# ndlongvn/MM-DTI

Measured on AMD Instinct MI355X. Metric: molecules/sec fwd+bwd (InfoNCE fine-tune), higher is better.
Workload: dtype fp16 forward / bf16 backward GEMM operands, fp32 accumulation

## Files before the change

include/mmdti_hip.h:

```cpp
#ifndef MMDTI_HIP_H
#define MMDTI_HIP_H

#ifdef __cplusplus
extern "C" {
#endif

typedef void* mmdti_stream_t;

#define MMDTI_OK 0
#define MMDTI_ERR_INVALID 1
#define MMDTI_ERR_LAUNCH 2

#define MMDTI_ACT_NONE 0
#define MMDTI_ACT_GELU 1
#define MMDTI_ACT_GELU_BWD 2
#define MMDTI_ACT_GELU_G 4
#define MMDTI_ACT_MUL_AUX 5

#define MMDTI_DT_F32 0
#define MMDTI_DT_BF16 1
#define MMDTI_DT_F32_ATOMIC 2
#define MMDTI_DT_F16 3
#define MMDTI_DT_AB_F16 16
#define MMDTI_DT_B_F16 32
// ... 113 lines not shown
                         long long arena_bytes, long long stats_bytes, void* ws, long long ws_bytes, long long dw_slab_bytes,
                         int fwd_f16);


int mmdti_layernorm_fwd(mmdti_stream_t stream, const float* x, const float* gamma, const float* beta, float eps,
                        int rows, int D, float* y_f32, void* y_bf16, float* mean, float* rstd,
                        const unsigned char* row_zero, float drop_p, unsigned long long seed, unsigned int site,
                        int y16_f16 );
int mmdti_layernorm_bwd(mmdti_stream_t stream, const void* dy, int dy_dtype, const float* dy_add, const float* x, const float* gamma,
                        const float* mean, const float* rstd, int rows, int D, const float* dres, float* dx,
                        float* dgamma, float* dbeta, const unsigned char* row_zero, float drop_p,
                        unsigned long long seed, unsigned int site, void* dx_bf16, float drop2_p, unsigned int site2,
                        float* dx_colsum);

int mmdti_colsum_bf16(mmdti_stream_t stream, const void* x_bf16, int rows, int cols, int ld, float* out);
int mmdti_cast_f32_bf16(mmdti_stream_t stream, const float* x, void* y_bf16, long long n, float drop_p,
                        unsigned long long seed, unsigned int site);
int mmdti_cast_bf16_f32(mmdti_stream_t stream, const void* x_bf16, float* y, long long n);
int mmdti_cast_f32_f16(mmdti_stream_t stream, const float* x, void* y_f16, long long n, float drop_p, unsigned long long seed,
                       unsigned int site);
int mmdti_cast_f16_bf16(mmdti_stream_t stream, const void* x_f16, int rows, int cols, int ldx, void* y_bf16);
int mmdti_dropout_f32(mmdti_stream_t stream, const float* x, float* y, long long n, float drop_p,
                      unsigned long long seed, unsigned int site);
int mmdti_axpy_f32(mmdti_stream_t stream, const float* x, float* y, long long n, float a);

int mmdti_embedding_fwd(mmdti_stream_t stream, const long long* ids, const float* table, long long n, int D,
                        int vocab, float* out, int accumulate);
int mmdti_embedding_bwd(mmdti_stream_t stream, const long long* ids, const float* dout, long long n, int D,
                        int vocab, long long padding_idx, float* dtable);
int mmdti_embedding_fwd3(mmdti_stream_t stream, const long long* ids_a, const float* table_a, int vocab_a, const long long* ids_b,
                         const float* table_b, int vocab_b, const long long* ids_c, const float* table_c, int vocab_c, long long n, int D,
                         float* out);
int mmdti_onehot_bf16(mmdti_stream_t stream, const long long* ids, long long n, int vocab, int ld, long long padding_idx,
                      void* out_bf16);
int mmdti_roberta_position_ids(mmdti_stream_t stream, const long long* ids, int B, int L, long long pad_idx,
                               long long* out);

int mmdti_gbf_features_fwd(mmdti_stream_t stream, const float* dist, const long long* edge_type, const float* mul,
                           const float* bias, const float* means, const float* stds, long long P, int K, int E,
                           void* feat_bf16);
int mmdti_gbf_features_bwd(mmdti_stream_t stream, const float* dist, const long long* edge_type, const float* mul,
                           const float* bias, const float* means, const float* stds, long long P, int K, int E,
                           const void* dfeat_bf16, float* dmul, float* dbias, float* dmeans, float* dstds);
int mmdti_gbf_bias_fwd(mmdti_stream_t stream, const float* dist, const void* edge_type,
                       int edge_bytes , const float* mul,
                       const float* bias, const float* means, const float* stds, const void* w1_bf16, const float* b1,
// ... 129 lines not shown
```

mm-dti_amd/csrc/elementwise.hip:

```cpp
#include "common.h"
#include <stdarg.h>
#include <stdio.h>

namespace mmdti {

static thread_local char g_err[512] = "";
void set_error(const char* fmt, ...) {
  va_list ap;
  va_start(ap, fmt);
  vsnprintf(g_err, sizeof(g_err), fmt, ap);
  va_end(ap);
}

static inline int grid_for(long long n, int per_block) {
  long long b = (n + per_block - 1) / per_block;
  if (b > 256 * 16) b = 256 * 16;
  if (b < 1) b = 1;
  return (int)b;
}

__device__ __forceinline__ bf16_t f2h16(float f) { return f2h_sat(f); }

template <bool F16>
__global__ __launch_bounds__(256) void cast_f32_bf16_kernel(const float* __restrict__ x, bf16_t* __restrict__ y,
// ... 32 lines not shown
    const int c = (int)(i - row * cols8) * 8;
    const uint4 u = *reinterpret_cast<const uint4*>(x + row * ldx + c);
    const uint32_t w[4] = {u.x, u.y, u.z, u.w};
    uint32_t o[4];
#pragma unroll
    for (int e = 0; e < 4; ++e) {
      const float lo = (float)__builtin_bit_cast(_Float16, (uint16_t)(w[e] & 0xffffu)), hi = (float)__builtin_bit_cast(_Float16, (uint16_t)(w[e] >> 16));
      o[e] = (uint32_t)f2bf(lo) | ((uint32_t)f2bf(hi) << 16);
    }
    *reinterpret_cast<uint4*>(y + row * (long long)cols8 * 8 + c) = make_uint4(o[0], o[1], o[2], o[3]);
  }
}

__global__ __launch_bounds__(256) void cast_bf16_f32_kernel(const bf16_t* __restrict__ x, float* __restrict__ y, long long n) {
  for (long long i = (long long)blockIdx.x * 256 + threadIdx.x; i < n; i += (long long)gridDim.x * 256) y[i] = bf2f(x[i]);
}

__global__ __launch_bounds__(256) void dropout_f32_kernel(const float* __restrict__ x, float* __restrict__ y, long long n,
                                                          uint32_t thresh, float dscale, uint64_t seed, uint32_t site) {
  for (long long i = (long long)blockIdx.x * 256 + threadIdx.x; i < n; i += (long long)gridDim.x * 256) {
    float o = x[i];
    if (thresh) o = dropout_keep(seed, site, (uint64_t)i, thresh) ? o * dscale : 0.f;
    y[i] = o;
  }
}

__global__ __launch_bounds__(256) void axpy_kernel(const float* __restrict__ x, float* __restrict__ y, long long n, float a) {
  for (long long i = (long long)blockIdx.x * 256 + threadIdx.x; i < n; i += (long long)gridDim.x * 256) y[i] += a * x[i];
}

__global__ __launch_bounds__(256) void gelu_bf16_kernel(const bf16_t* __restrict__ u, bf16_t* __restrict__ y, long long n) {
  for (long long i = (long long)blockIdx.x * 256 + threadIdx.x; i < n; i += (long long)gridDim.x * 256)
    y[i] = f2bf(gelu_erf(bf2f(u[i])));
}

__global__ __launch_bounds__(256) void colsum_bf16_kernel(const bf16_t* __restrict__ x, int rows, int cols, int ld,
                                                          float* __restrict__ out) {
  __shared__ float red[8][256 + 8];
  const int cc = threadIdx.x & 31, rl = threadIdx.x >> 5;
  const int c0 = blockIdx.x * 256 + cc * 8;
  float acc[8] = {0, 0, 0, 0, 0, 0, 0, 0};
  if (c0 < cols) {
    const int rstep = gridDim.y * 8;
    int r = blockIdx.y * 8 + rl;
    if (c0 + 8 <= cols) {
      for (; r + 3 * rstep < rows; r += 4 * rstep) {
// ... 546 lines not shown
                     (bf16_t*)y_bf16, n8);
  MMDTI_LAUNCH_CHECK();
  return MMDTI_OK;
}

extern "C" int mmdti_cast_bf16_f32(mmdti_stream_t stream, const void* x_bf16, float* y, long long n) {
  MMDTI_REQUIRE(x_bf16 && y && n > 0, "cast_bf16_f32: bad arguments");
  hipLaunchKernelGGL(cast_bf16_f32_kernel, dim3(grid_for(n, 256)), dim3(256), 0, (hipStream_t)stream,
                     (const bf16_t*)x_bf16, y, n);
  MMDTI_LAUNCH_CHECK();
  return MMDTI_OK;
}

extern "C" int mmdti_dropout_f32(mmdti_stream_t stream, const float* x, float* y, long long n, float drop_p,
                                 unsigned long long seed, unsigned int site) {
  MMDTI_REQUIRE(x && y && n > 0, "dropout_f32: bad arguments");
  DROP_SETUP("dropout_f32");
  hipLaunchKernelGGL(dropout_f32_kernel, dim3(grid_for(n, 256)), dim3(256), 0, (hipStream_t)stream, x, y, n, th, sc,
                     (uint64_t)seed, (uint32_t)site);
  MMDTI_LAUNCH_CHECK();
  return MMDTI_OK;
}

extern "C" int mmdti_axpy_f32(mmdti_stream_t stream, const float* x, float* y, long long n, float a) {
  MMDTI_REQUIRE(x && y && n > 0, "axpy_f32: bad arguments");
  hipLaunchKernelGGL(axpy_kernel, dim3(grid_for(n, 256)), dim3(256), 0, (hipStream_t)stream, x, y, n, a);
  MMDTI_LAUNCH_CHECK();
  return MMDTI_OK;
}

extern "C" int mmdti_gelu_fwd_bf16(mmdti_stream_t stream, const void* u_bf16, void* y_bf16, long long n) {
  MMDTI_REQUIRE(u_bf16 && y_bf16 && n > 0, "gelu_fwd_bf16: bad arguments");
  hipLaunchKernelGGL(gelu_bf16_kernel, dim3(grid_for(n, 256)), dim3(256), 0, (hipStream_t)stream,
                     (const bf16_t*)u_bf16, (bf16_t*)y_bf16, n);
  MMDTI_LAUNCH_CHECK();
  return MMDTI_OK;
}

extern "C" int mmdti_colsum_bf16(mmdti_stream_t stream, const void* x_bf16, int rows, int cols, int ld, float* out) {
  MMDTI_REQUIRE(x_bf16 && out && rows > 0 && cols > 0 && ld >= cols, "colsum_bf16: bad arguments");
  MMDTI_REQUIRE(ld % 8 == 0 && aligned16(x_bf16), "colsum_bf16: ld%%8 and 16-byte alignment required");
  int gy = cdiv(rows, 8 * 8);
  if (gy > 1024) gy = 1024;
  hipLaunchKernelGGL(colsum_bf16_kernel, dim3(cdiv(cols, 256), gy), dim3(256), 0, (hipStream_t)stream,
                     (const bf16_t*)x_bf16, rows, cols, ld, out);
  MMDTI_LAUNCH_CHECK();
// ... 239 lines not shown
```

mm-dti_amd/mmdti_hip/functional.py:

```python
from __future__ import annotations

import ctypes
import os
import weakref

import math
from types import SimpleNamespace
from typing import List, Optional

import torch

from . import ops, paths
from .ops import BF16, F32
from .runtime import fused_views, wbf16, wfwd, gbuf, dropout_state, notify_grads_ready
from .freeze import layer_trainable, plan_tower, trainable_flags


def _lin_bwd_params(dy_bf16, x_bf16, weight, bias, rows=None, bias_done=False):
    gw = gbuf(weight)
    gb = gbuf(bias) if (bias is not None and not bias_done) else None
    if gw is not None:
        ops.linear_bwd_weight(dy_bf16, x_bf16, gw, rows=rows, db=gb if (gb is not None and gb.numel() == gw.shape[0]) else None)
        if gb is not None and gb.numel() == gw.shape[0]:
            gb = None
# ... 1018 lines not shown
    @staticmethod
    def backward(ctx, dout):
        st, mod = ctx.st, ctx.mod
        if getattr(st, "consumed", False):
            raise ops.MMDTIError("RobertaEncoderFn: backward through the same forward twice (retain_graph) is not supported")
        st.consumed = True
        B, Lq, D = st.B, st.Lq, st.D
        dx = dout.contiguous().view(st.Mq, D)
        if st.stack is not None:
            dx = _bert_stack_bwd(st, dx)
            notify_grads_ready(st.stack.T.params)
            st.stack = None
        plan = st.plan
        for li, layer, L in zip(range(len(st.layers) - 1, -1, -1), reversed(list(mod.layers)), reversed(st.layers)):
            if li < plan.lowest:
                L.__dict__.clear()
                continue
            dx, _ = _bert_layer_bwd(st, L, dx, st.seed, (plan.needs_dx(li), False))
            L.__dict__.clear()
            notify_grads_ready(layer.parameters())
        if not plan.below:
            _join_stream_after_backward()
            return None, None, None, None, None, None
        de = ops.layernorm_bwd(dx, st.e.view(st.Mq, D), mod.emb_ln_w, st.em, st.er, gbuf(mod.emb_ln_w), gbuf(mod.emb_ln_b),
                               drop_p=st.p_hid, seed=st.seed, site=st.site_emb)
        cfg = mod.cfg
        de16 = ops.cast_bf16(de)
        for ids, w, pad in ((st.ids, mod.word, cfg.pad_idx), (st.pos, mod.position, cfg.pad_idx), (None, mod.token_type, -1)):
            g = gbuf(w)
            if g is not None:
                if ids is None:
                    ids = st.ids if w.shape[0] == 1 else torch.zeros_like(st.ids)
                ops.embedding_bwd_gemm(ids, de16, g, pad)
        notify_grads_ready(mod.embeddings.parameters())
        _join_stream_after_backward()
        return None, None, None, None, None, None


class CrossLayerFn(torch.autograd.Function):

    @staticmethod
    def forward(ctx, s1, s2, key_add, layer, cfg, training, packs=None, anchor=None):
        seed = dropout_state.next_seed()
        sites = _Sites()
        p_hid = cfg.hidden_dropout if training else 0.0
        p_att = cfg.attn_dropout if training else 0.0
        if packs is not None:
            vl = ops.AttnVarlen(packs[0], packs[1])
            D = s1.shape[-1]
            st = SimpleNamespace(B=packs[0].B, Lq=vl.Lq, Lk=vl.Lk, D=D, seed=seed, Mq=vl.q_rows, Mk=vl.k_rows, vl=vl)
        else:
            B, Lq, D = s1.shape
            Lk = s2.shape[1]
            st = SimpleNamespace(B=B, Lq=Lq, Lk=Lk, D=D, seed=seed, Mq=B * Lq, Mk=B * Lk, vl=None)
        s1c = s1.contiguous().view(st.Mq, D)
        s1_16 = ops.cast_act16(s1c)
        s2_16 = ops.cast_act16(s2.contiguous().view(st.Mk, D))
        L, out32, _ = _bert_layer_fwd(st, s1c, s1_16, s2_16, None if key_add is None else key_add.contiguous(), bert_weights(layer), cfg.heads,
                                      p_hid, p_att, cfg.ln_eps, seed, sites, False)
        if any(ctx.needs_input_grad):
            ctx.st, ctx.L, ctx.layer = st, L, layer
        ctx.shapes = (s1.shape, s2.shape)
        return out32.view(s1.shape)

    @staticmethod
    def backward(ctx, dout):
        st, L = ctx.st, ctx.L
        want = ctx.needs_input_grad[:2]
        ds1, ds2 = _bert_layer_bwd(st, L, dout.contiguous().view(st.Mq, st.D), st.seed, want)
        L.__dict__.clear()
        notify_grads_ready(ctx.layer.parameters())
        return (None if ds1 is None else ds1.view(ctx.shapes[0]), None if ds2 is None else ds2.view(ctx.shapes[1]), None, None, None, None, None,
                None)


class DropoutFn(torch.autograd.Function):

    @staticmethod
    def forward(ctx, x, p, training):
        if not training or p == 0.0:
            ctx.p = 0.0
            return x
        ctx.p, ctx.seed = p, dropout_state.next_seed()
        return ops.dropout_f32(x.contiguous(), p, ctx.seed, 1)

    @staticmethod
    def backward(ctx, d):
        if ctx.p == 0.0:
            return d, None, None
        return ops.dropout_f32(d.contiguous(), ctx.p, ctx.seed, 1), None, None


def _pad8(n):
    return (n + 7) // 8 * 8


class InfoNCEFn(torch.autograd.Function):

    @staticmethod
    def forward(ctx, query, positive, mod, training, gather, reduce_scatter, row0, packs=None, anchor=None):
        if packs is not None:
            B, D = packs[0].B, query.shape[-1]
            Nq, Np = packs[0].M, packs[1].M
            if not (POOL_THEN_PROJECT and mod.info_proj_query[0].weight.shape[0] % 8 == 0 and mod.info_proj_positive[0].weight.shape[0] % 8 == 0):
                raise ops.MMDTIError("InfoNCEFn: packed rows need the pool-then-project form (hidden width % 8 == 0)")
        else:
            B, Nq, D = query.shape
            Np = positive.shape[1]
        d = mod.d_l
        ldp = _pad8(d)
        seed = dropout_state.next_seed()
        p = mod.embed_dropout if training else 0.0
        st = SimpleNamespace(B=B, Nq=Nq, Np=Np, D=D, d=d, ldp=ldp, seed=seed, p=p)
        dev = query.device

        def proj(x, seq, n, dropout_p, site, pack=None):
            L = SimpleNamespace()
            rows = B * n if pack is None else pack.M
            L.x16 = ops.cast_act16(x.contiguous().view(rows, D), dropout_p, seed, site)
            L.u = torch.empty(rows, seq[0].weight.shape[0], device=dev, dtype=BF16)
            h = ops.linear_fwd(L.x16, wfwd(seq[0].weight), seq[0].bias, act=ops.ACT_GELU_FWD, aux_out=L.u, out_dtype=BF16)
            Hd = h.shape[1]
            if pack is not None:
                L.hbar = ops.seq_mean_packed_fwd(h, pack, Hd, Hd)
                L.mean = ops.linear_f32_fwd(L.hbar, seq[2].weight.detach(), seq[2].bias.detach())
                L.h = None
                return L
            if POOL_THEN_PROJECT and Hd % 8 == 0:
                L.hbar = ops.seq_mean_fwd(h, B, n, Hd, Hd)
                L.mean = ops.linear_f32_fwd(L.hbar, seq[2].weight.detach(), seq[2].bias.detach())
                L.h = None
                return L
            L.h = h
            pr = torch.zeros(B * n, ldp, device=dev, dtype=BF16)
# ... 22 lines not shown
    @staticmethod
    def backward(ctx, dloss):
        st, mod = ctx.st, ctx.mod
        B, d, ldp = st.B, st.d, st.ldp
        dq = ops.l2norm_bwd(st.dqh, st.qh, st.qinv)
        dk = ops.l2norm_bwd(st.dkh, st.kh, st.kinv)
        dboth = torch.cat((dq, dk), dim=1)
        if ctx.rs is not None:
            dboth = ctx.rs(dboth)
        dboth = (dboth * dloss).contiguous()

        def proj_bwd(L, dmean, seq, n, dropout_p, site, want_dx, pack=None):
            if L.h is None:
                gw, gb = gbuf(seq[2].weight), gbuf(seq[2].bias)
                dhbar = ops.linear_f32_bwd(L.hbar, seq[2].weight.detach(), None, dmean.contiguous(), gw, gb)
                Hd = L.hbar.shape[1]
                if pack is not None:
                    du = ops.seq_mean_packed_bwd(dhbar, pack, Hd, Hd, aux=L.u, aux_mode=1 if ops.GELU_SAVE_GRAD else 2)
                else:
                    du = ops.seq_mean_bwd(dhbar, B, n, Hd, Hd, aux=L.u, aux_mode=1 if ops.GELU_SAVE_GRAD else 2)
                _lin_bwd_params(du, L.x16, seq[0].weight, seq[0].bias)
                if not want_dx:
                    return None
                dx = ops.linear_bwd_input(du, wbf16(seq[0].weight), out_dtype=F32)
                if dropout_p > 0:
                    dx = ops.dropout_f32(dx, dropout_p, st.seed, site)
                return dx
            dpr = ops.seq_mean_bwd(dmean.contiguous(), B, n, d, ldp)
            gw = gbuf(seq[2].weight)
            if gw is not None:
                ops.linear_bwd_weight(dpr, L.h, gw)
            gb = gbuf(seq[2].bias)
            if gb is not None:
                ops.colsum(dpr, gb, cols=d)
            du = ops.gemm(dpr, wbf16(seq[2].weight), M=B * n, N=L.h.shape[1], K=d, lda=ldp, ldb=seq[2].weight.shape[1], transB=True,
                          act=ops.ACT_GELU_DX, aux_in=L.u)
            _lin_bwd_params(du, L.x16, seq[0].weight, seq[0].bias)
            if not want_dx:
                return None
            dx = ops.linear_bwd_input(du, wbf16(seq[0].weight), out_dtype=F32)
            if dropout_p > 0:
                dx = ops.dropout_f32(dx, dropout_p, st.seed, site)
            return dx

        pk = st.packs
        dxq = proj_bwd(st.Lq, dboth[:, :d], mod.info_proj_query, st.Nq, st.p, 1, ctx.needs_input_grad[0], None if pk is None else pk[0])
        dxp = proj_bwd(st.Lp, dboth[:, d:], mod.info_proj_positive, st.Np, 0.0, 2, ctx.needs_input_grad[1], None if pk is None else pk[1])
        notify_grads_ready(mod.parameters())
        if pk is not None:
            return dxq, dxp, None, None, None, None, None, None, None
        return (None if dxq is None else dxq.view(B, st.Nq, st.D), None if dxp is None else dxp.view(B, st.Np, st.D), None, None, None, None, None, None,
                None)


class InfoNCELossFn(torch.autograd.Function):

    @staticmethod
    def forward(ctx, q, k, temperature):
        B, d = q.shape
        qh, qinv = ops.l2norm_fwd(q.contiguous())
        kh, kinv = ops.l2norm_fwd(k.contiguous())
        loss = torch.zeros(1, device=q.device, dtype=F32)
        dqh, dkh = torch.zeros_like(qh), torch.zeros_like(kh)
        ops.infonce_dir(qh, kh, 0, B, temperature, loss, dqh, dkh)
        ops.infonce_dir(kh, qh, 0, B, temperature, loss, dkh, dqh)
        ctx.sv = (qh, qinv, kh, kinv, dqh, dkh)
        return (loss / (2.0 * B)).view(())

    @staticmethod
    def backward(ctx, dl):
        qh, qinv, kh, kinv, dqh, dkh = ctx.sv
        return ops.l2norm_bwd(dqh, qh, qinv) * dl, ops.l2norm_bwd(dkh, kh, kinv) * dl, None


class CTLossFn(torch.autograd.Function):
# ... 106 lines not shown
```

mm-dti_amd/mmdti_hip/models/bert_layers.py:

```python
import json
import os
from types import SimpleNamespace

import torch
import torch.nn as nn

from ..unicore_compat import LayerNorm
from ..functional import RobertaEncoderFn, CrossLayerFn
from ..freeze import grad_anchor


class _SelfAttnParams(nn.Module):
    def __init__(self, dim):
        super().__init__()
        self.query = nn.Linear(dim, dim)
        self.key = nn.Linear(dim, dim)
        self.value = nn.Linear(dim, dim)


class _SelfOutputParams(nn.Module):
    def __init__(self, in_dim, dim, eps):
        super().__init__()
        self.dense = nn.Linear(in_dim, dim)
        self.LayerNorm = LayerNorm(dim, eps=eps)
# ... 11 lines not shown
        super().__init__()
        self.dense = nn.Linear(dim, ffn)


class BertLayerParams(nn.Module):
    def __init__(self, dim, ffn, eps):
        super().__init__()
        self.attention = _AttentionParams(dim, eps)
        self.intermediate = _IntermediateParams(dim, ffn)
        self.output = _SelfOutputParams(ffn, dim, eps)


class BertCrossEncoder(nn.Module):

    def __init__(self, config, layer_num):
        super().__init__()
        if config.hidden_act != "gelu":
            raise NotImplementedError("only hidden_act='gelu' is on the MM-DTI path")
        self.cfg = SimpleNamespace(heads=config.num_attention_heads, ln_eps=config.layer_norm_eps,
                                   hidden_dropout=config.hidden_dropout_prob, attn_dropout=config.attention_probs_dropout_prob)
        self.layer = nn.ModuleList([BertLayerParams(config.hidden_size, config.intermediate_size, config.layer_norm_eps)
                                    for _ in range(layer_num)])

    def forward(self, s1_hidden_states, s2_hidden_states, s2_attention_mask, output_all_encoded_layers=True, packs=None):
        if packs is None:
            B, Lk = s2_hidden_states.shape[0], s2_hidden_states.shape[1]
            key_add = s2_attention_mask.reshape(B, Lk).float()
        else:
            key_add = None
        outs = []
        for layer in self.layer:
            s1_hidden_states = CrossLayerFn.apply(s1_hidden_states.float(), s2_hidden_states.float(), key_add, layer, self.cfg, self.training, packs,
                                                  grad_anchor(layer.parameters()))
            if output_all_encoded_layers:
                outs.append(s1_hidden_states)
        if not output_all_encoded_layers:
            outs.append(s1_hidden_states)
        return outs


class _RobertaEmbeddings(nn.Module):
    def __init__(self, cfg):
        super().__init__()
        self.word_embeddings = nn.Embedding(cfg.vocab, cfg.dim, padding_idx=cfg.pad_idx)
        self.position_embeddings = nn.Embedding(cfg.max_pos, cfg.dim, padding_idx=cfg.pad_idx)
        self.token_type_embeddings = nn.Embedding(cfg.type_vocab, cfg.dim)
        self.LayerNorm = LayerNorm(cfg.dim, eps=cfg.ln_eps)


class _RobertaEncoder(nn.Module):
    def __init__(self, cfg):
        super().__init__()
        self.layer = nn.ModuleList([BertLayerParams(cfg.dim, cfg.ffn, cfg.ln_eps) for _ in range(cfg.layers)])


class _Pooler(nn.Module):
# ... 80 lines not shown
```

mm-dti_amd/mmdti_hip/models/infonce.py:

```python
import torch
from torch import nn

from ..functional import InfoNCEFn, InfoNCELossFn
from ..freeze import grad_anchor


class InfoNCE(nn.Module):
    def __init__(self, bert_output_size, graph_ouput_size, temperature=0.1, reduction='mean', negative_mode='unpaired'):
        super().__init__()
        self.temperature = temperature
        self.reduction = reduction
        self.negative_mode = negative_mode
        self.orig_d_l = bert_output_size
        self.orig_d_av = graph_ouput_size
        self.d_l, self.d_av = 50, 50
        self.embed_dropout = 0.1
        self.training = True
        self.info_proj_query = nn.Sequential(nn.Linear(self.orig_d_l, self.orig_d_l), nn.GELU(), nn.Linear(self.orig_d_l, self.d_l))
        self.info_proj_positive = nn.Sequential(nn.Linear(self.orig_d_av, self.orig_d_av), nn.GELU(), nn.Linear(self.orig_d_av, self.d_av))
        self._gather = None
        self._reduce_scatter = None
        self._row0 = 0

    def set_global_negatives(self, gather, reduce_scatter, row0):
        self._gather, self._reduce_scatter, self._row0 = gather, reduce_scatter, int(row0)

    def forward(self, query, positive_key, negative_keys=None, packs=None):
        if packs is not None:
            if negative_keys is not None or self.reduction != 'mean' or query.dim() != 2 or positive_key.dim() != 2 or packs[0].B != packs[1].B:
                raise ValueError('packed rows: <query> / <positive_key> must be [rows, dim] with one packing each, implicit negatives.')
            return InfoNCEFn.apply(query.float(), positive_key.float(), self, self.training, self._gather, self._reduce_scatter, self._row0, packs,
                                   grad_anchor(self.parameters()))
        if negative_keys is not None:
            raise ValueError("explicit negative_keys are unreachable in the reference (infonce.py:98 raises); not supported")
        if self.reduction != 'mean':
            raise ValueError("only reduction='mean' is on the MM-DTI path")
        if self.orig_d_l == self.d_l or self.orig_d_av == self.d_av:
            raise ValueError("identity projection (input width == 50) is not on the MM-DTI path")
        if query.dim() != 3 or positive_key.dim() != 3:
            raise ValueError('<query> and <positive_key> must be [batch, seq, dim] token representations.')
        if len(query) != len(positive_key):
            raise ValueError('<query> and <positive_key> must must have the same number of samples.')
        return InfoNCEFn.apply(query.float(), positive_key.float(), self, self.training, self._gather, self._reduce_scatter, self._row0, None,
                               grad_anchor(self.parameters()))


def info_nce(query, positive_key, negative_keys=None, temperature=0.1, reduction='mean', negative_mode='unpaired'):
    if query.dim() != 2:
        raise ValueError('<query> must have 2 dimensions.')
    if positive_key.dim() != 2:
        raise ValueError('<positive_key> must have 2 dimensions.')
    if negative_keys is not None:
        if negative_mode == 'unpaired' and negative_keys.dim() != 2:
            raise ValueError("<negative_keys> must have 2 dimensions if <negative_mode> == 'unpaired'.")
        if negative_mode == 'paired' and negative_keys.dim() != 3:
            raise ValueError("<negative_keys> must have 3 dimensions if <negative_mode> == 'paired'.")
    if len(query) != len(positive_key):
        raise ValueError('<query> and <positive_key> must must have the same number of samples.')
    if negative_keys is not None:
        if negative_mode == 'paired' and len(query) != len(negative_keys):
            raise ValueError("If negative_mode == 'paired', then <negative_keys> must have the same number of samples as <query>.")
    if query.shape[-1] != positive_key.shape[-1]:
        raise ValueError('Vectors of <query> and <positive_key> should have the same number of components.')
    if negative_keys is not None:
        if query.shape[-1] != negative_keys.shape[-1]:
            raise ValueError('Vectors of <query> and <negative_keys> should have the same number of components.')
        raise ValueError("explicit negative_keys: the reference's symmetric cross-entropy (infonce.py:98) raises for "
# ... 5 lines not shown
```

mm-dti_amd/mmdti_hip/models/mm_model.py:

```python
from __future__ import annotations

import argparse
import itertools
import os
from types import SimpleNamespace

import torch
import torch.nn as nn

from ..unicore_compat import Dictionary, init_bert_params, get_activation_fn
from ..functional import PairBiasFn, PairCompactFn, EmbeddingFn, DropoutFn, MaskedPoolFn, LinearF32Fn
from .. import ops
from ..freeze import grad_anchor
from ..collate import right_pad, collate_batch
from ..packing import PackedRows

PAIR_RAGGED = os.environ.get("MMDTI_PAIR_RAGGED", "1") != "0"
from .transformers import TransformerEncoderWithPair
from .bert_layers import BertCrossEncoder, RobertaTower
from .infonce import InfoNCE
from .fds import FDS

BACKBONE = {'transformer': TransformerEncoderWithPair}


def pad_1d_tokens(values, pad_idx):
    return right_pad(values, pad_idx)


def pad_2d(values, pad_idx):
    return right_pad(values, pad_idx, square=True)


def pad_coords(values, pad_idx):
    return right_pad(values, pad_idx, tail=(3,))

# ... 51 lines not shown

def fds_config():
    return SimpleNamespace(feature_dim=512, bucket_num=20, bucket_start=0, start_update=0, start_smooth=1, kernel='gaussian',
                           ks=5, sigma=1, momentum=0.9, col_data="expt", raw_data="")


def crossmodal_config():
    return SimpleNamespace(attention_probs_dropout_prob=0.2, gradient_checkpointing=False, hidden_act="gelu",
                           hidden_dropout_prob=0.3, hidden_size=512, initializer_range=0.02, intermediate_size=2048,
                           layer_norm_eps=1e-12, max_position_embeddings=512, num_attention_heads=16, num_hidden_layers=12,
                           position_embedding_type="absolute")


class CrossAttentionModel(nn.Module):

    def __init__(self, cross_cfg, num_layers=1):
        super().__init__()
        self.text_attention = BertCrossEncoder(cross_cfg, num_layers)
        self.graph_attention = BertCrossEncoder(cross_cfg, num_layers)
        self.dropout = nn.Dropout(cross_cfg.hidden_dropout_prob)
        self.two_streams = os.environ.get("MMDTI_CROSS_TWO_STREAMS", "1") != "0"
        self._stream = None

    def forward(self, text_embeddings, graph_embeddings, text_mask, graph_mask, packs=None):
        text_embeddings = DropoutFn.apply(text_embeddings, self.dropout.p, self.training)
        graph_embeddings = DropoutFn.apply(graph_embeddings, self.dropout.p, self.training)
        if packs is not None:
            rev = (packs[1], packs[0])
            if self.two_streams and text_embeddings.is_cuda:
                main = torch.cuda.current_stream()
                if self._stream is None:
                    self._stream = torch.cuda.Stream()
                st = self._stream
                st.wait_stream(main)
                with torch.cuda.stream(st):
                    text_to_graph = self.text_attention(text_embeddings, graph_embeddings, None, packs=packs)[-1]
                for t in (text_embeddings, graph_embeddings):
                    t.record_stream(st)
                graph_to_text = self.graph_attention(graph_embeddings, text_embeddings, None, packs=rev)[-1]
                main.wait_stream(st)
                text_to_graph.record_stream(main)
                return text_to_graph, graph_to_text
            graph_to_text = self.graph_attention(graph_embeddings, text_embeddings, None, packs=rev)[-1]
            text_to_graph = self.text_attention(text_embeddings, graph_embeddings, None, packs=packs)[-1]
            return text_to_graph, graph_to_text
        extended_txt_mask = (1.0 - text_mask.unsqueeze(1).unsqueeze(2).to(dtype=torch.float32)) * -10000.0
        extended_img_mask = (1.0 - graph_mask.unsqueeze(1).unsqueeze(2).to(dtype=torch.float32)) * -10000.0
        if self.two_streams and text_embeddings.is_cuda:
            main = torch.cuda.current_stream()
            if self._stream is None:
                self._stream = torch.cuda.Stream()
            st = self._stream
            st.wait_stream(main)
            with torch.cuda.stream(st):
                text_to_graph = self.text_attention(text_embeddings, graph_embeddings, extended_img_mask)[-1]
            for t in (text_embeddings, graph_embeddings, extended_img_mask):
                t.record_stream(st)
            graph_to_text = self.graph_attention(graph_embeddings, text_embeddings, extended_txt_mask)[-1]
            main.wait_stream(st)
            text_to_graph.record_stream(main)
            return text_to_graph, graph_to_text
        graph_to_text = self.graph_attention(graph_embeddings, text_embeddings, extended_txt_mask)[-1]
        text_to_graph = self.text_attention(text_embeddings, graph_embeddings, extended_img_mask)[-1]
        return text_to_graph, graph_to_text


class MM_Model(nn.Module):
    def __init__(self, output_dim=2, **params):
        super().__init__()
        self.cross_cfg = params.get('_cross_cfg') or crossmodal_config()
        self.fds_cfg = fds_config()
        self.args = params.get('_mol_args') or molecule_architecture()
        self.output_dim = output_dim
        self.data_type = 'molecule'
        self.remove_hs = params.get('remove_hs', False)
        self.use_fds = params.get('fds', False)
        self.using_scale = params.get('use_scaler', True)
        self.fds_num = params.get('fds_num', 30)
        self.fds_raw_path = params.get('fds_raw_path', '')
        self.fds_col_data = params.get('fds_col_data', '')
        self.ct_w = params.get('ct_w', 0.2)
        self.task = params.get('task', False)
        self.chemberta_dir = params.get('chemberta_dir', '')
        self.unimol_dir = params.get('unimol_dir', '')

        dictionary = params.get('_dictionary')
# ... 156 lines not shown
            main = torch.cuda.current_stream()
            side.wait_stream(main)
            with torch.cuda.stream(side):
                out_bert = self.bert(input_ids, attention_mask, return_dict=True, pack=pk2)[0]

        if pk1 is None:
            xs = EmbeddingFn.apply(self.embed_tokens.weight, src_tokens, self.padding_idx)
            bias_s = self.pair_bias(src_distance, src_edge_type, kt_host)
            encoder_rep = self.encoder.encode(xs, bias_s, padding_mask, key_tiles)[0]
        else:
            ids1, pad1 = src_tokens.reshape(-1)[pk1.gather], padding_mask.reshape(-1)[pk1.gather]
            xs = EmbeddingFn.apply(self.embed_tokens.weight, ids1, self.padding_idx)
            bias_s = self.pair_bias(src_distance, src_edge_type, kt_host, pk1.rows_host)
            if bias_s.dtype != torch.float16:
                bias_s = PairCompactFn.apply(bias_s, src_tokens.shape[1])
            encoder_rep = self.encoder.encode(xs, bias_s, pad1, key_tiles, pack=pk1)[0]

        if side is not None:
            main.wait_stream(side)
            out_bert.record_stream(main)
        else:
            out_bert = self.bert(input_ids, attention_mask, return_dict=True, pack=pk2)[0]

        infonce_side = False
        if return_infonce_loss:
            if side is not None and self.infonce_on_side_stream:
                side.wait_stream(main)
                with torch.cuda.stream(side):
                    ct_loss = self.infonce(encoder_rep, out_bert, packs=packs)
                encoder_rep.record_stream(side)
                out_bert.record_stream(side)
                infonce_side = True
            else:
                ct_loss = self.infonce(encoder_rep, out_bert, packs=packs)

        cross_txt_output_layer, cross_output_layer = self.cross_modal_module(encoder_rep, out_bert, img_mask, attention_mask, packs=packs)
        classification_feats_pooled = MaskedPoolFn.apply(cross_txt_output_layer, cross_output_layer, img_mask, attention_mask, packs)

        smoothed_features = classification_feats_pooled
        if self.training and epoch >= self.fds_cfg.start_smooth and self.use_fds and self.task == 'regression':
            smoothed_features = self.FDS.smooth(smoothed_features, net_target, epoch)
            classification_feats_pooled = smoothed_features

        logits = self.classification_head(smoothed_features)

        rnc_loss = None
        if return_ct_loss and net_target is not None:
            if use_weight:
                rnc_loss = self.CT(classification_feats_pooled, net_target, logits, weights=weights, w=self.ct_w)
            else:
                rnc_loss = self.CT(classification_feats_pooled, net_target, logits, w=self.ct_w)
        if infonce_side:
            main.wait_stream(side)
            ct_loss.record_stream(main)
        out = [logits]
        if return_feature:
            out.append(classification_feats_pooled)
        if return_infonce_loss:
            out.append(ct_loss)
# ... 7 lines not shown
```

mm-dti_amd/mmdti_hip/ops.py:

```python
from __future__ import annotations

import os

import torch

from ._abi import lib, MMDTIError

BF16 = torch.bfloat16
F32 = torch.float32
F16 = torch.float16

ACT_NONE, ACT_GELU, ACT_GELU_BWD, ACT_TANH, ACT_GELU_G, ACT_MUL_AUX = 0, 1, 2, 3, 4, 5
GELU_SAVE_GRAD = os.environ.get("MMDTI_GELU_SAVE_GRAD", "1") != "0"
GBF_FULL_BWD = os.environ.get("MMDTI_GBF_FULL_BWD", "1") != "0"
ACT_GELU_FWD = ACT_GELU_G if GELU_SAVE_GRAD else ACT_GELU
ACT_GELU_DX = ACT_MUL_AUX if GELU_SAVE_GRAD else ACT_GELU_BWD
DT_F32, DT_BF16, DT_F32_ATOMIC, DT_F16, DT_AB_F16, DT_B_F16 = 0, 1, 2, 3, 16, 32

FWD_F16 = os.environ.get("MMDTI_FWD_FP16", "1") != "0"


def set_forward_fp16(on: bool):
    global FWD_F16
    FWD_F16 = bool(on)
# ... 101 lines not shown
    if not linear_ln_eligible(x, w, residual):
        y = linear_fwd(x, w, bias, residual=residual, out_dtype=F32, drop_p=drop_p, seed=seed, site=site)
        h32, h16, mean, rstd = layernorm_fwd(y, gamma, beta, eps, want_f32=want_f32, want_bf16=want_bf16)
        return y, h32, h16, mean, rstd
    _chk16(x, "linear_ln.x", contiguous=False); _chk16(w, "linear_ln.w", contiguous=False)
    if x.dtype != w.dtype:
        raise MMDTIError("linear_ln_fwd: x and w must share one 16-bit type")
    M, K = x.shape
    N = w.shape[0]
    y = torch.empty(M, N, device=x.device, dtype=F32)
    h32 = torch.empty(M, N, device=x.device, dtype=F32) if want_f32 else None
    h16 = torch.empty(M, N, device=x.device, dtype=act16()) if want_bf16 else None
    mean = torch.empty(M, device=x.device, dtype=F32)
    rstd = torch.empty(M, device=x.device, dtype=F32)
    t0 = kernel_timer.begin("gemm")
    lib().mmdti_gemm_ln_bf16(_stream(), x.data_ptr(), w.data_ptr(), _p(bias), _p(residual), M, N, K, x.stride(0), w.stride(0),
                             N if residual is None else residual.stride(0), float(drop_p), int(seed), int(site), y.data_ptr(), gamma.data_ptr(),
                             beta.data_ptr(), float(eps), _p(h32), _p(h16), mean.data_ptr(), rstd.data_ptr(),
                             (1 if x.dtype == F16 else 0) | (2 if (h16 is not None and h16.dtype == F16) else 0))
    kernel_timer.end("gemm", t0, 2.0 * M * N * K, tag=(M, N, K, 0, 0, 1, 1, "ln", want_bf16, want_f32, residual is not None))
    return y, h32, h16, mean, rstd


def linear_bwd_input(dy, w, *, act=ACT_NONE, aux_in=None, out_dtype=BF16, K_valid=None, colsum=None):
    M, N = dy.shape
    K = w.shape[1]
    return gemm(dy, w, M=M, N=K, K=(N if K_valid is None else K_valid), lda=dy.stride(0), ldb=w.stride(0), transB=True, act=act, aux_in=aux_in,
                out_dtype=out_dtype, colsum=colsum)


def _splitk_for(M, N, K):
    tiles = ((M + 127) // 128) * ((N + 127) // 128)
    ktiles = (K + 63) // 64
    sk = max(256 // tiles, min(8, max(1, 2048 // tiles)))
    return max(1, min(ktiles, sk))


DW_BIAS = os.environ.get("MMDTI_DW_BIAS", "1") != "0"
SPLITK_SLABS = os.environ.get("MMDTI_SPLITK_SLABS", "1") != "0"


def linear_bwd_weight(dy, x, dw, *, rows=None, db=None):
    M = dy.shape[0] if rows is None else rows
    N, K = dw.shape
    if x.dtype == F16 and (x.dim() != 2 or x.stride(1) != 1):
        x = x.contiguous().view(-1, x.shape[-1])
    if db is not None:
        _chk(db, F32, "linear_bwd_weight.db")
        if not DW_BIAS:
            colsum(dy, db, cols=N)
            db = None
# ... 110 lines not shown
    if x.dtype != F16:
        return x
    if x.dim() != 2 or x.stride(1) != 1:
        x = x.contiguous().view(-1, x.shape[-1])
    y = torch.empty(x.shape, device=x.device, dtype=BF16)
    lib().mmdti_cast_f16_bf16(_stream(), x.data_ptr(), x.shape[0], x.shape[1], x.stride(0), y.data_ptr())
    return y


def cast_f32(x):
    _chk(x, BF16, "cast_f32.x")
    y = torch.empty(x.shape, device=x.device, dtype=F32)
    lib().mmdti_cast_bf16_f32(_stream(), x.data_ptr(), y.data_ptr(), x.numel())
    return y


def dropout_f32(x, p, seed, site):
    _chk(x, F32, "dropout_f32.x")
    if p == 0.0:
        return x
    y = torch.empty_like(x)
    lib().mmdti_dropout_f32(_stream(), x.data_ptr(), y.data_ptr(), x.numel(), float(p), int(seed), int(site))
    return y


def axpy_(y, x, a=1.0):
    lib().mmdti_axpy_f32(_stream(), x.data_ptr(), y.data_ptr(), x.numel(), float(a))
    return y


def embedding_fwd(ids, table, out=None, accumulate=False):
    _chk(ids, torch.int64, "embedding.ids")
    _chk(table, F32, "embedding.table")
    V, D = table.shape
    if out is None:
        out = torch.empty(*ids.shape, D, device=table.device, dtype=F32)
    lib().mmdti_embedding_fwd(_stream(), ids.data_ptr(), table.data_ptr(), ids.numel(), D, V, out.data_ptr(), int(accumulate))
    return out


def embedding_fwd3(ids_a, table_a, ids_b, table_b, table_c, ids_c=None):
    _chk(ids_a, torch.int64, "embedding.ids_a"); _chk(ids_b, torch.int64, "embedding.ids_b")
    for t in (table_a, table_b, table_c):
        _chk(t, F32, "embedding.table")
    D = table_a.shape[1]
    out = torch.empty(*ids_a.shape, D, device=table_a.device, dtype=F32)
# ... 688 lines not shown
```

Before: 4950.

## Fuse cross-modal input dropout, 16-bit casts and gradient fan-in into one kernel

Adds a vectorized dropout_fanin kernel that sums up to three fp32 inputs, applies dropout and writes fp32 and/or fp16/bf16 outputs in one pass. A new FusionInputFn produces the dropped fp32 tensor and its 16-bit copy once per modality, so the cross layers reuse it instead of recasting. In backward it merges the gradient branches in a single pass. The InfoNCE projection backward folds its dropout into the GEMM epilogue, and the embedding LN backward emits bf16 directly. The dropout seed plumbing changes, so the random masks differ from the previous per-module DropoutFn path.

```diff
diff --git a/include/mmdti_hip.h b/include/mmdti_hip.h
--- a/include/mmdti_hip.h
+++ b/include/mmdti_hip.h
@@ -159,6 +159,8 @@
 int mmdti_cast_f16_bf16(mmdti_stream_t stream, const void* x_f16, int rows, int cols, int ldx, void* y_bf16);
 int mmdti_dropout_f32(mmdti_stream_t stream, const float* x, float* y, long long n, float drop_p,
                       unsigned long long seed, unsigned int site);
+int mmdti_dropout_fanin_f32(mmdti_stream_t stream, const float* a, const float* b, const float* c, float* y_f32, void* y16, int y16_f16,
+                            long long n, float drop_p, unsigned long long seed, unsigned int site);
 int mmdti_axpy_f32(mmdti_stream_t stream, const float* x, float* y, long long n, float a);
 
 int mmdti_embedding_fwd(mmdti_stream_t stream, const long long* ids, const float* table, long long n, int D,
diff --git a/mm-dti_amd/csrc/elementwise.hip b/mm-dti_amd/csrc/elementwise.hip
--- a/mm-dti_amd/csrc/elementwise.hip
+++ b/mm-dti_amd/csrc/elementwise.hip
@@ -78,6 +78,52 @@
     float o = x[i];
     if (thresh) o = dropout_keep(seed, site, (uint64_t)i, thresh) ? o * dscale : 0.f;
     y[i] = o;
+  }
+}
+
+template <bool F16>
+__global__ __launch_bounds__(256) void dropout_fanin_kernel(const float* __restrict__ a, const float* __restrict__ b, const float* __restrict__ c,
+                                                            float* __restrict__ y32, bf16_t* __restrict__ y16, long long n4, long long n,
+                                                            uint32_t thresh, float dscale, uint64_t seed, uint32_t site) {
+#pragma clang fp contract(off)
+  for (long long i = (long long)blockIdx.x * 256 + threadIdx.x; i < n4; i += (long long)gridDim.x * 256) {
+    const float4 v = reinterpret_cast<const float4*>(a)[i];
+    float o[4] = {v.x, v.y, v.z, v.w};
+    if (b) {
+      const float4 w = reinterpret_cast<const float4*>(b)[i];
+      o[0] += w.x; o[1] += w.y; o[2] += w.z; o[3] += w.w;
+    }
+    if (thresh) {
+      const Rand4 r = philox4(seed, site, (uint64_t)i);
+      const uint32_t rw[4] = {r.x, r.y, r.z, r.w};
+#pragma unroll
+      for (int e = 0; e < 4; ++e) o[e] = rw[e] >= thresh ? o[e] * dscale : 0.f;
+    }
+    if (c) {
+      const float4 w = reinterpret_cast<const float4*>(c)[i];
+      o[0] += w.x; o[1] += w.y; o[2] += w.z; o[3] += w.w;
+    }
+    if (y32) reinterpret_cast<float4*>(y32)[i] = make_float4(o[0], o[1], o[2], o[3]);
+    if (y16) {
+      uint2 pk;
+      if (F16) {
+        pk.x = (uint32_t)f2h16(o[0]) | ((uint32_t)f2h16(o[1]) << 16);
+        pk.y = (uint32_t)f2h16(o[2]) | ((uint32_t)f2h16(o[3]) << 16);
+      } else {
+        pk.x = (uint32_t)f2bf(o[0]) | ((uint32_t)f2bf(o[1]) << 16);
+        pk.y = (uint32_t)f2bf(o[2]) | ((uint32_t)f2bf(o[3]) << 16);
+      }
+      reinterpret_cast<uint2*>(y16)[i] = pk;
+    }
+  }
+  if (blockIdx.x == 0 && threadIdx.x < (n & 3)) {
+    const long long i = (n & ~3LL) + threadIdx.x;
+    float o = a[i];
+    if (b) o += b[i];
+    if (thresh) o = dropout_keep(seed, site, (uint64_t)i, thresh) ? o * dscale : 0.f;
+    if (c) o += c[i];
+    if (y32) y32[i] = o;
+    if (y16) y16[i] = F16 ? f2h16(o) : f2bf(o);
   }
 }
 
@@ -670,6 +716,24 @@
   return MMDTI_OK;
 }
 
+extern "C" int mmdti_dropout_fanin_f32(mmdti_stream_t stream, const float* a, const float* b, const float* c, float* y_f32, void* y16,
+                                       int y16_f16, long long n, float drop_p, unsigned long long seed, unsigned int site) {
+  MMDTI_REQUIRE(a && (y_f32 || y16) && n > 0, "dropout_fanin_f32: bad arguments");
+  MMDTI_REQUIRE(aligned16(a) && (!b || aligned16(b)) && (!c || aligned16(c)) && (!y_f32 || aligned16(y_f32)) &&
+                    (reinterpret_cast<uintptr_t>(y16) & 7) == 0,
+                "dropout_fanin_f32: alignment");
+  DROP_SETUP("dropout_fanin_f32");
+  const dim3 grid(grid_for(n / 4 + 1, 256)), block(256);
+  if (y16_f16)
+    hipLaunchKernelGGL(dropout_fanin_kernel<true>, grid, block, 0, (hipStream_t)stream, a, b, c, y_f32, (bf16_t*)y16, n / 4, n, th, sc,
+                       (uint64_t)seed, (uint32_t)site);
+  else
+    hipLaunchKernelGGL(dropout_fanin_kernel<false>, grid, block, 0, (hipStream_t)stream, a, b, c, y_f32, (bf16_t*)y16, n / 4, n, th, sc,
+                       (uint64_t)seed, (uint32_t)site);
+  MMDTI_LAUNCH_CHECK();
+  return MMDTI_OK;
+}
+
 extern "C" int mmdti_axpy_f32(mmdti_stream_t stream, const float* x, float* y, long long n, float a) {
   MMDTI_REQUIRE(x && y && n > 0, "axpy_f32: bad arguments");
   hipLaunchKernelGGL(axpy_kernel, dim3(grid_for(n, 256)), dim3(256), 0, (hipStream_t)stream, x, y, n, a);
diff --git a/mm-dti_amd/mmdti_hip/functional.py b/mm-dti_amd/mmdti_hip/functional.py
--- a/mm-dti_amd/mmdti_hip/functional.py
+++ b/mm-dti_amd/mmdti_hip/functional.py
@@ -1064,10 +1064,9 @@
         if not plan.below:
             _join_stream_after_backward()
             return None, None, None, None, None, None
-        de = ops.layernorm_bwd(dx, st.e.view(st.Mq, D), mod.emb_ln_w, st.em, st.er, gbuf(mod.emb_ln_w), gbuf(mod.emb_ln_b),
-                               drop_p=st.p_hid, seed=st.seed, site=st.site_emb)
+        _, de16 = ops.layernorm_bwd(dx, st.e.view(st.Mq, D), mod.emb_ln_w, st.em, st.er, gbuf(mod.emb_ln_w), gbuf(mod.emb_ln_b),
+                                    drop_p=st.p_hid, seed=st.seed, site=st.site_emb, bf16_copy=(0.0, 0))
         cfg = mod.cfg
-        de16 = ops.cast_bf16(de)
         for ids, w, pad in ((st.ids, mod.word, cfg.pad_idx), (st.pos, mod.position, cfg.pad_idx), (None, mod.token_type, -1)):
             g = gbuf(w)
             if g is not None:
@@ -1082,7 +1081,7 @@
 class CrossLayerFn(torch.autograd.Function):
 
     @staticmethod
-    def forward(ctx, s1, s2, key_add, layer, cfg, training, packs=None, anchor=None):
+    def forward(ctx, s1, s2, key_add, layer, cfg, training, packs=None, anchor=None, s1_16=None, s2_16=None):
         seed = dropout_state.next_seed()
         sites = _Sites()
         p_hid = cfg.hidden_dropout if training else 0.0
@@ -1096,8 +1095,10 @@
             Lk = s2.shape[1]
             st = SimpleNamespace(B=B, Lq=Lq, Lk=Lk, D=D, seed=seed, Mq=B * Lq, Mk=B * Lk, vl=None)
         s1c = s1.contiguous().view(st.Mq, D)
-        s1_16 = ops.cast_act16(s1c)
-        s2_16 = ops.cast_act16(s2.contiguous().view(st.Mk, D))
+        s1_16 = ops.cast_act16(s1c) if s1_16 is None else s1_16.view(st.Mq, D)
+        s2_16 = ops.cast_act16(s2.contiguous().view(st.Mk, D)) if s2_16 is None else s2_16.view(st.Mk, D)
+        if s1_16.dtype != ops.act16() or s2_16.dtype != ops.act16():
+            raise ops.MMDTIError("CrossLayerFn: the 16-bit operands are not of the forward GEMM input type")
         L, out32, _ = _bert_layer_fwd(st, s1c, s1_16, s2_16, None if key_add is None else key_add.contiguous(), bert_weights(layer), cfg.heads,
                                       p_hid, p_att, cfg.ln_eps, seed, sites, False)
         if any(ctx.needs_input_grad):
@@ -1113,7 +1114,34 @@
         L.__dict__.clear()
         notify_grads_ready(ctx.layer.parameters())
         return (None if ds1 is None else ds1.view(ctx.shapes[0]), None if ds2 is None else ds2.view(ctx.shapes[1]), None, None, None, None, None,
-                None)
+                None, None, None)
+
+
+class FusionInputFn(torch.autograd.Function):
+
+    @staticmethod
+    def forward(ctx, x, p, training, seed):
+        ctx.p = p if training else 0.0
+        ctx.seed = seed
+        xc = x.contiguous()
+        if ctx.p == 0.0:
+            y, y16 = xc, ops.dropout_fanin(xc, want_f32=False, want_16=True)[1]
+        else:
+            y, y16 = ops.dropout_fanin(xc, p=ctx.p, seed=seed, site=1, want_16=True)
+        ctx.mark_non_differentiable(y16)
+        ctx.set_materialize_grads(False)
+        return x.view_as(x), y.view_as(y), y.view_as(y), y16
+
+    @staticmethod
+    def backward(ctx, d_direct, d_a, d_b, _):
+        parts = [d.contiguous() for d in (d_a, d_b) if d is not None]
+        if not parts:
+            return d_direct, None, None, None
+        if len(parts) == 1 and ctx.p == 0.0 and d_direct is None:
+            return parts[0], None, None, None
+        dx, _ = ops.dropout_fanin(parts[0], parts[1] if len(parts) > 1 else None, None if d_direct is None else d_direct.contiguous(),
+                                  p=ctx.p, seed=ctx.seed, site=1)
+        return dx, None, None, None
 
 
 class DropoutFn(torch.autograd.Function):
@@ -1140,7 +1168,7 @@
 class InfoNCEFn(torch.autograd.Function):
 
     @staticmethod
-    def forward(ctx, query, positive, mod, training, gather, reduce_scatter, row0, packs=None, anchor=None):
+    def forward(ctx, query, positive, mod, training, gather, reduce_scatter, row0, packs=None, anchor=None, seed=None):
         if packs is not None:
             B, D = packs[0].B, query.shape[-1]
             Nq, Np = packs[0].M, packs[1].M
@@ -1151,7 +1179,8 @@
             Np = positive.shape[1]
         d = mod.d_l
         ldp = _pad8(d)
-        seed = dropout_state.next_seed()
+        if seed is None:
+            seed = dropout_state.next_seed()
         p = mod.embed_dropout if training else 0.0
         st = SimpleNamespace(B=B, Nq=Nq, Np=Np, D=D, d=d, ldp=ldp, seed=seed, p=p)
         dev = query.device
@@ -1220,10 +1249,7 @@
                 _lin_bwd_params(du, L.x16, seq[0].weight, seq[0].bias)
                 if not want_dx:
                     return None
-                dx = ops.linear_bwd_input(du, wbf16(seq[0].weight), out_dtype=F32)
-                if dropout_p > 0:
-                    dx = ops.dropout_f32(dx, dropout_p, st.seed, site)
-                return dx
+                return ops.linear_bwd_input(du, wbf16(seq[0].weight), out_dtype=F32, drop_p=dropout_p, seed=st.seed, site=site)
             dpr = ops.seq_mean_bwd(dmean.contiguous(), B, n, d, ldp)
             gw = gbuf(seq[2].weight)
             if gw is not None:
@@ -1236,19 +1262,16 @@
             _lin_bwd_params(du, L.x16, seq[0].weight, seq[0].bias)
             if not want_dx:
                 return None
-            dx = ops.linear_bwd_input(du, wbf16(seq[0].weight), out_dtype=F32)
-            if dropout_p > 0:
-                dx = ops.dropout_f32(dx, dropout_p, st.seed, site)
-            return dx
+            return ops.linear_bwd_input(du, wbf16(seq[0].weight), out_dtype=F32, drop_p=dropout_p, seed=st.seed, site=site)
 
         pk = st.packs
         dxq = proj_bwd(st.Lq, dboth[:, :d], mod.info_proj_query, st.Nq, st.p, 1, ctx.needs_input_grad[0], None if pk is None else pk[0])
         dxp = proj_bwd(st.Lp, dboth[:, d:], mod.info_proj_positive, st.Np, 0.0, 2, ctx.needs_input_grad[1], None if pk is None else pk[1])
         notify_grads_ready(mod.parameters())
         if pk is not None:
-            return dxq, dxp, None, None, None, None, None, None, None
+            return dxq, dxp, None, None, None, None, None, None, None, None
         return (None if dxq is None else dxq.view(B, st.Nq, st.D), None if dxp is None else dxp.view(B, st.Np, st.D), None, None, None, None, None, None,
-                None)
+                None, None)
 
 
 class InfoNCELossFn(torch.autograd.Function):
diff --git a/mm-dti_amd/mmdti_hip/models/bert_layers.py b/mm-dti_amd/mmdti_hip/models/bert_layers.py
--- a/mm-dti_amd/mmdti_hip/models/bert_layers.py
+++ b/mm-dti_amd/mmdti_hip/models/bert_layers.py
@@ -57,16 +57,16 @@
         self.layer = nn.ModuleList([BertLayerParams(config.hidden_size, config.intermediate_size, config.layer_norm_eps)
                                     for _ in range(layer_num)])
 
-    def forward(self, s1_hidden_states, s2_hidden_states, s2_attention_mask, output_all_encoded_layers=True, packs=None):
+    def forward(self, s1_hidden_states, s2_hidden_states, s2_attention_mask, output_all_encoded_layers=True, packs=None, s1_16=None, s2_16=None):
         if packs is None:
             B, Lk = s2_hidden_states.shape[0], s2_hidden_states.shape[1]
             key_add = s2_attention_mask.reshape(B, Lk).float()
         else:
             key_add = None
         outs = []
-        for layer in self.layer:
+        for li, layer in enumerate(self.layer):
             s1_hidden_states = CrossLayerFn.apply(s1_hidden_states.float(), s2_hidden_states.float(), key_add, layer, self.cfg, self.training, packs,
-                                                  grad_anchor(layer.parameters()))
+                                                  grad_anchor(layer.parameters()), s1_16 if li == 0 else None, s2_16)
             if output_all_encoded_layers:
                 outs.append(s1_hidden_states)
         if not output_all_encoded_layers:
diff --git a/mm-dti_amd/mmdti_hip/models/infonce.py b/mm-dti_amd/mmdti_hip/models/infonce.py
--- a/mm-dti_amd/mmdti_hip/models/infonce.py
+++ b/mm-dti_amd/mmdti_hip/models/infonce.py
@@ -25,12 +25,12 @@
     def set_global_negatives(self, gather, reduce_scatter, row0):
         self._gather, self._reduce_scatter, self._row0 = gather, reduce_scatter, int(row0)
 
-    def forward(self, query, positive_key, negative_keys=None, packs=None):
+    def forward(self, query, positive_key, negative_keys=None, packs=None, seed=None):
         if packs is not None:
             if negative_keys is not None or self.reduction != 'mean' or query.dim() != 2 or positive_key.dim() != 2 or packs[0].B != packs[1].B:
                 raise ValueError('packed rows: <query> / <positive_key> must be [rows, dim] with one packing each, implicit negatives.')
             return InfoNCEFn.apply(query.float(), positive_key.float(), self, self.training, self._gather, self._reduce_scatter, self._row0, packs,
-                                   grad_anchor(self.parameters()))
+                                   grad_anchor(self.parameters()), seed)
         if negative_keys is not None:
             raise ValueError("explicit negative_keys are unreachable in the reference (infonce.py:98 raises); not supported")
         if self.reduction != 'mean':
@@ -42,7 +42,7 @@
         if len(query) != len(positive_key):
             raise ValueError('<query> and <positive_key> must must have the same number of samples.')
         return InfoNCEFn.apply(query.float(), positive_key.float(), self, self.training, self._gather, self._reduce_scatter, self._row0, None,
-                               grad_anchor(self.parameters()))
+                               grad_anchor(self.parameters()), seed)
 
 
 def info_nce(query, positive_key, negative_keys=None, temperature=0.1, reduction='mean', negative_mode='unpaired'):
diff --git a/mm-dti_amd/mmdti_hip/models/mm_model.py b/mm-dti_amd/mmdti_hip/models/mm_model.py
--- a/mm-dti_amd/mmdti_hip/models/mm_model.py
+++ b/mm-dti_amd/mmdti_hip/models/mm_model.py
@@ -9,9 +9,10 @@
 import torch.nn as nn
 
 from ..unicore_compat import Dictionary, init_bert_params, get_activation_fn
-from ..functional import PairBiasFn, PairCompactFn, EmbeddingFn, DropoutFn, MaskedPoolFn, LinearF32Fn
+from ..functional import PairBiasFn, PairCompactFn, EmbeddingFn, DropoutFn, FusionInputFn, MaskedPoolFn, LinearF32Fn
 from .. import ops
 from ..freeze import grad_anchor
+from ..runtime import dropout_state
 from ..collate import right_pad, collate_batch
 from ..packing import PackedRows
 
@@ -109,46 +110,61 @@
         self.two_streams = os.environ.get("MMDTI_CROSS_TWO_STREAMS", "1") != "0"
         self._stream = None
 
+    def fuse_inputs(self, text_embeddings, graph_embeddings):
+        sides = []
+        for t in (text_embeddings, graph_embeddings):
+            live = self.training and self.dropout.p != 0.0
+            x, s1, s2, h16 = FusionInputFn.apply(t.float(), self.dropout.p, self.training, dropout_state.next_seed() if live else 0)
+            sides.append(SimpleNamespace(x=x, s1=s1, s2=s2, h16=h16))
+        return sides
+
     def forward(self, text_embeddings, graph_embeddings, text_mask, graph_mask, packs=None):
-        text_embeddings = DropoutFn.apply(text_embeddings, self.dropout.p, self.training)
-        graph_embeddings = DropoutFn.apply(graph_embeddings, self.dropout.p, self.training)
+        if torch.is_tensor(text_embeddings):
+            text_embeddings, graph_embeddings = self.fuse_inputs(text_embeddings, graph_embeddings)
+        text, graph = text_embeddings, graph_embeddings
+
+        def t2g(mask):
+            return self.text_attention(text.s1, graph.s2, mask, packs=packs, s1_16=text.h16, s2_16=graph.h16)[-1]
+
+        def g2t(mask, pk):
+            return self.graph_attention(graph.s1, text.s2, mask, packs=pk, s1_16=graph.h16, s2_16=text.h16)[-1]
         if packs is not None:
             rev = (packs[1], packs[0])
-            if self.two_streams and text_embeddings.is_cuda:
+            if self.two_streams and text.s1.is_cuda:
                 main = torch.cuda.current_stream()
                 if self._stream is None:
                     self._stream = torch.cuda.Stream()
                 st = self._stream
                 st.wait_stream(main)
                 with torch.cuda.stream(st):
-                    text_to_graph = self.text_attention(text_embeddings, graph_embeddings, None, packs=packs)[-1]
-                for t in (text_embeddings, graph_embeddings):
+                    text_to_graph = t2g(None)
+                for t in (text.s1, graph.s2, text.h16, graph.h16):
                     t.record_stream(st)
-                graph_to_text = self.graph_attention(graph_embeddings, text_embeddings, None, packs=rev)[-1]
+                graph_to_text = g2t(None, rev)
                 main.wait_stream(st)
                 text_to_graph.record_stream(main)
                 return text_to_graph, graph_to_text
-            graph_to_text = self.graph_attention(graph_embeddings, text_embeddings, None, packs=rev)[-1]
-            text_to_graph = self.text_attention(text_embeddings, graph_embeddings, None, packs=packs)[-1]
+            graph_to_text = g2t(None, rev)
+            text_to_graph = t2g(None)
             return text_to_graph, graph_to_text
         extended_txt_mask = (1.0 - text_mask.unsqueeze(1).unsqueeze(2).to(dtype=torch.float32)) * -10000.0
         extended_img_mask = (1.0 - graph_mask.unsqueeze(1).unsqueeze(2).to(dtype=torch.float32)) * -10000.0
-        if self.two_streams and text_embeddings.is_cuda:
+        if self.two_streams and text.s1.is_cuda:
             main = torch.cuda.current_stream()
             if self._stream is None:
                 self._stream = torch.cuda.Stream()
             st = self._stream
             st.wait_stream(main)
             with torch.cuda.stream(st):
-                text_to_graph = self.text_attention(text_embeddings, graph_embeddings, extended_img_mask)[-1]
-            for t in (text_embeddings, graph_embeddings, extended_img_mask):
+                text_to_graph = t2g(extended_img_mask)
+            for t in (text.s1, graph.s2, text.h16, graph.h16, extended_img_mask):
                 t.record_stream(st)
-            graph_to_text = self.graph_attention(graph_embeddings, text_embeddings, extended_txt_mask)[-1]
+            graph_to_text = g2t(extended_txt_mask, None)
             main.wait_stream(st)
             text_to_graph.record_stream(main)
             return text_to_graph, graph_to_text
-        graph_to_text = self.graph_attention(graph_embeddings, text_embeddings, extended_txt_mask)[-1]
-        text_to_graph = self.text_attention(text_embeddings, graph_embeddings, extended_img_mask)[-1]
+        graph_to_text = g2t(extended_txt_mask, None)
+        text_to_graph = t2g(extended_img_mask)
         return text_to_graph, graph_to_text
 
 
@@ -351,19 +367,22 @@
         else:
             out_bert = self.bert(input_ids, attention_mask, return_dict=True, pack=pk2)[0]
 
+        nce_seed = dropout_state.next_seed() if return_infonce_loss else None
+        fused = self.cross_modal_module.fuse_inputs(encoder_rep, out_bert)
+        encoder_rep, out_bert = fused[0].x, fused[1].x
         infonce_side = False
         if return_infonce_loss:
             if side is not None and self.infonce_on_side_stream:
                 side.wait_stream(main)
                 with torch.cuda.stream(side):
-                    ct_loss = self.infonce(encoder_rep, out_bert, packs=packs)
+                    ct_loss = self.infonce(encoder_rep, out_bert, packs=packs, seed=nce_seed)
                 encoder_rep.record_stream(side)
                 out_bert.record_stream(side)
                 infonce_side = True
             else:
-                ct_loss = self.infonce(encoder_rep, out_bert, packs=packs)
-
-        cross_txt_output_layer, cross_output_layer = self.cross_modal_module(encoder_rep, out_bert, img_mask, attention_mask, packs=packs)
+                ct_loss = self.infonce(encoder_rep, out_bert, packs=packs, seed=nce_seed)
+
+        cross_txt_output_layer, cross_output_layer = self.cross_modal_module(fused[0], fused[1], img_mask, attention_mask, packs=packs)
         classification_feats_pooled = MaskedPoolFn.apply(cross_txt_output_layer, cross_output_layer, img_mask, attention_mask, packs)
 
         smoothed_features = classification_feats_pooled
diff --git a/mm-dti_amd/mmdti_hip/ops.py b/mm-dti_amd/mmdti_hip/ops.py
--- a/mm-dti_amd/mmdti_hip/ops.py
+++ b/mm-dti_amd/mmdti_hip/ops.py
@@ -147,11 +147,11 @@
     return y, h32, h16, mean, rstd
 
 
-def linear_bwd_input(dy, w, *, act=ACT_NONE, aux_in=None, out_dtype=BF16, K_valid=None, colsum=None):
+def linear_bwd_input(dy, w, *, act=ACT_NONE, aux_in=None, out_dtype=BF16, K_valid=None, colsum=None, drop_p=0.0, seed=0, site=0):
     M, N = dy.shape
     K = w.shape[1]
     return gemm(dy, w, M=M, N=K, K=(N if K_valid is None else K_valid), lda=dy.stride(0), ldb=w.stride(0), transB=True, act=act, aux_in=aux_in,
-                out_dtype=out_dtype, colsum=colsum)
+                out_dtype=out_dtype, colsum=colsum, drop_p=drop_p, seed=seed, site=site)
 
 
 def _splitk_for(M, N, K):
@@ -308,6 +308,22 @@
     y = torch.empty_like(x)
     lib().mmdti_dropout_f32(_stream(), x.data_ptr(), y.data_ptr(), x.numel(), float(p), int(seed), int(site))
     return y
+
+
+def dropout_fanin(a, b=None, c=None, *, p=0.0, seed=0, site=0, want_f32=True, want_16=False):
+    _chk(a, F32, "dropout_fanin.a")
+    for t, nm in ((b, "b"), (c, "c")):
+        if t is not None:
+            _chk(t, F32, "dropout_fanin." + nm)
+            if t.shape != a.shape:
+                raise MMDTIError(f"dropout_fanin: {nm} is {tuple(t.shape)}, a is {tuple(a.shape)}")
+    if not (want_f32 or want_16):
+        raise MMDTIError("dropout_fanin: no output requested")
+    y32 = torch.empty_like(a) if want_f32 else None
+    y16 = torch.empty(a.shape, device=a.device, dtype=act16()) if want_16 else None
+    lib().mmdti_dropout_fanin_f32(_stream(), a.data_ptr(), _p(b), _p(c), _p(y32), _p(y16), int(y16 is not None and y16.dtype == F16), a.numel(),
+                                  float(p), int(seed), int(site))
+    return y32, y16
 
 
 def axpy_(y, x, a=1.0):
```

Result: no change. 4990 (median of 6 runs) (+0.8%).
